# sailist/emotion-recognition-in-conversation

Measured on AMD Instinct MI355X. Metric: utterances/sec training step, COGMEN IEMOCAP-6 atv, higher is better.
Workload: dtype bf16

## Files before the change

### emotion-recognition-in-conversation_amd/capi.py

```python
import ctypes as C
import os
import re
import subprocess

import torch

_HERE = os.path.dirname(os.path.abspath(__file__))
LIB_PATH = os.environ.get("ERC_LIB_PATH") or os.path.join(_HERE, "lib", "libercgraft.so")
CSRC = os.path.join(_HERE, "csrc")
HEADER = os.path.join(os.path.dirname(_HERE), "include", "ercgraft.h")


class ErcGraftError(RuntimeError):
    pass


_CTYPES = {"int": C.c_int, "int32_t": C.c_int, "int64_t": C.c_int64, "uint64_t": C.c_uint64, "float": C.c_float}


def _ctype(decl, proto, ret=False):
    t = " ".join(decl.replace("*", " * ").split())
    if ret and t == "const char *":
        return C.c_char_p
    if "*" in t:
# ... 741 lines not shown


def enc_transpose_bf16(X, ldx, R, Cn, YT, ldyt, plain=None, ldp=0):
    _call("erc_enc_transpose_bf16", X, 1 if X.dtype == torch.float32 else 0, ldx, R, Cn, YT, ldyt, plain, ldp)


def enc_colsum_ws_floats(Cn):
    return int(lib().erc_enc_colsum_ws_floats(Cn))


def enc_colsum(X, ldx, R, Cn, out, ws):
    _call("erc_enc_colsum", X, 1 if X.dtype == torch.bfloat16 else 0, ldx, R, Cn, out, ws)


def enc_inverse_rows(node_row, N, inv, n_rows):
    _call("erc_enc_inverse_rows", node_row, N, inv, n_rows)


def wgrad_bf16(table, n_desc, item_base, n_items, slabs, counters, terms=1):
    if terms > 1:
        _call("erc_wgrad_split", terms, table, n_desc, item_base, n_items, slabs, counters)
        return
    _call("erc_wgrad_bf16", table, n_desc, item_base, n_items, slabs, counters)


def wgrad_bf16_adam(table, n_desc, item_base, n_items, slabs, counters, n_tiles, p, g, m, v, n, lr, b1, b2, eps, wd, decoupled,
                    grad_scale, state, shadow_table, health, terms=1, p2p_desc=None):
    args = (table, n_desc, item_base, n_items, slabs, counters, int(n_tiles), p, g, m, v, n, lr, b1, b2, eps, wd, int(decoupled),
            grad_scale, state) + _shadow(shadow_table)
    if p2p_desc is not None:
        _call("erc_wgrad_adam_p2p", terms, *args, C.addressof(p2p_desc))
    elif terms > 1:
        _call("erc_wgrad_split_adam", terms, *args, health)
    else:
        _call("erc_wgrad_bf16_adam", *args, health)


def wgrad_bf16_wide(table, n_desc, wg_base, n_wgs, slabs, counters):
    _call("erc_wgrad_bf16_wide", table, n_desc, wg_base, n_wgs, slabs, counters)


def wgrad_bf16_set_spin_limit(limit):
    _call("erc_wgrad_bf16_set_spin_limit", int(limit))


def wgrad_bf16_set_stamps(t, item=0):
    _call("erc_wgrad_bf16_set_stamps", t, int(item))


def wgrad_bf16_slab_floats():
    return int(lib().erc_wgrad_bf16_slab_floats())


def wgrad_bf16_max_k_per_split():
    return int(lib().erc_wgrad_bf16_max_k_per_split())


def wgrad_slab_floats():
    return int(lib().erc_wgrad_slab_floats())


def wgrad_max_k_per_split():
    return int(lib().erc_wgrad_max_k_per_split())


def dgcn_tail_limits():
    return int(lib().erc_dgcn_tail_max_rows()), int(lib().erc_dgcn_tail_max_window())


def dgcn_tail_set_stamps(stamps):
    _call("erc_dgcn_tail_set_stamps", stamps)


def dgcn_tail_stats_floats(n_rows):
    return int(lib().erc_dgcn_tail_stats_floats(n_rows))


def dgcn_tail(slabs, n_slabs, slab_stride, rgcn_bias, g, window, W_rel, b_rel, W_root, W1, b1, W2, b2, labels, weight, n_classes,
              n_rows, drop_p, rng, Xc, ldx, Hc, AGG, Zc, logits, dlogits, dZc, dXc, lddx, dAGG, dHc, stats, n_dev=None, label_rows=None):
    args = (slabs, n_slabs, int(slab_stride), rgcn_bias, g["in_ptr"], g["in_src"], window, W_rel, b_rel, W_root, W1, b1, W2, b2,
            labels, weight, n_classes, n_rows, float(drop_p), rng, Xc, ldx, Hc, AGG, Zc, logits, dlogits, dZc, dXc, lddx, dAGG, dHc,
            stats)
    if n_dev is None and label_rows is None:
        _call("erc_dgcn_tail", *args)
    else:
        _call("erc_dgcn_tail_cap", *args, n_dev, label_rows)


def head_ce_stats_floats(n_rows):
    return int(lib().erc_head_ce_stats_floats(n_rows))


def head_ce(Z, ldz, F, Cn, n_rows, W, bias, labels, weight, mask_scale, logits, ldl, dlogits, lddl, dZ, lddz, stats):
    _call("erc_head_ce", Z, ldz, F, Cn, n_rows, W, bias, labels, weight, mask_scale, logits, ldl, dlogits, lddl, dZ, lddz,
          stats)


def cim_meta(lengths, B, T, n_cap, node_off, node_row):
    _call("erc_cim_meta", lengths, B, T, n_cap, node_off, node_row)


def gru_scan_fwd(GX, W_hhT, b_hh, lengths, node_off, B, T, rows, Hout, Hdrop, drop_p, rng, rng_stream, gates, ghn, Hprev):
    _call("erc_gru_scan_fwd", GX, W_hhT, b_hh, lengths, node_off, B, T, rows, Hout, Hdrop, drop_p, rng, rng_stream, gates, ghn,
          Hprev)


# ... 51 lines not shown
```

### emotion-recognition-in-conversation_amd/csrc/wgrad_bf16.hip

```cpp
#include "erc_common.h"
#include "optim_dev.h"
#include "split_dev.h"
#include <string.h>

namespace {

typedef float f32x4 __attribute__((ext_vector_type(4)));
typedef short bf16x8 __attribute__((ext_vector_type(8)));
typedef unsigned int u32x4 __attribute__((ext_vector_type(4)));
typedef unsigned int u32x2 __attribute__((ext_vector_type(2)));
#define ERC_GLOBAL __attribute__((address_space(1)))

constexpr int W2_IDX_CAP = 4096;
constexpr int W2_SLAB = 128 * 64 + 192;
constexpr int W2_MAX_DESC = 16;

struct W2Desc {
    const unsigned short* A;
    const unsigned short* B;
    float* C;
    float* bias_a;
    float* bias_b;
    const int32_t* b_gather;
    const int32_t* k_dev;
    int lda, ldb, ldc, M, N, K;
    int ct, cvec, splits, tiles_n, item_base, n_items, tile_base;
    int kind;
};

struct W2Adam {
    int decoupled, spin_limit;
    float lr, b1, b2, eps, wd, grad_scale;
    float *data, *grad, *m, *v;
    int64_t* state;
    unsigned short* shadow;
    const int32_t* skip;
    int32_t* seq;
    int32_t* health;
    ShadowTab tab;
    int x_world, x_rank, x_spin, x_pad;
    float* x_pub[8];
    int32_t* x_flags[8];
    int64_t* x_epoch;
    int64_t x_npad;
};
static_assert(sizeof(W2Desc) == 112, "W2Desc layout");

__device__ __forceinline__ float ld_sc1(const float* p) { return __hip_atomic_load(p, __ATOMIC_RELAXED, __HIP_MEMORY_SCOPE_AGENT); }
__device__ __forceinline__ void st_sc1(float* p, float v) { __hip_atomic_store(p, v, __ATOMIC_RELAXED, __HIP_MEMORY_SCOPE_AGENT); }
__device__ __forceinline__ void st_sc1_x4(float* p, f32x4 v) {
    asm volatile("global_store_dwordx4 %0, %1, off sc0 sc1\n\ts_nop 1" ::"v"(p), "v"(v) : "memory");
}
__device__ __forceinline__ f32x4 ld_sc1_x4(const float* p) {
    f32x4 v;
    asm volatile("global_load_dwordx4 %0, %1, off sc0 sc1" : "=v"(v) : "v"(p) : "memory");
    return v;
}
__device__ __forceinline__ float bf_lo(unsigned d) { return __builtin_bit_cast(float, d << 16); }
__device__ __forceinline__ float bf_hi(unsigned d) { return __builtin_bit_cast(float, d & 0xffff0000u); }
__device__ __forceinline__ unsigned perm_lo(unsigned x, unsigned y) { return __builtin_amdgcn_perm(y, x, 0x05040100u); }
__device__ __forceinline__ unsigned perm_hi(unsigned x, unsigned y) { return __builtin_amdgcn_perm(y, x, 0x07060302u); }

#define W2_STAMP(slot)                                                                          \
    do {                                                                                        \
        if (stamps && threadIdx.x == 0) stamps[slot] = __builtin_amdgcn_s_memrealtime();        \
    } while (0)

template <bool ADAM, bool WIDE, int NT>
__device__ __forceinline__ void w2_body(const W2Desc& d, const int local, float* red, float* bred, int* idx, int* s_flag,
                                        float* slabs, int* counters, uint64_t* stamps_item, uint64_t* stamps_tile, const W2Adam& ad) {
    uint64_t* stamps = stamps_item;
    W2_STAMP(0);
    bool adam_on = false;
    int64_t adam_step = 0;
    AdamCoef ac;
    if (ADAM && d.kind == 1) {
        const bool skip = ad.skip && __hip_atomic_load(ad.skip, __ATOMIC_RELAXED, __HIP_MEMORY_SCOPE_AGENT) != 0;
        adam_step = ad.state[4 + blockIdx.x] + 1;
        adam_on = !skip;
        ac.init(ad.lr, ad.b1, ad.b2, ad.eps, ad.wd, ad.decoupled, ad.grad_scale, adam_step);
    }
    auto bump_step = [&]() __attribute__((always_inline)) {
        if (!ADAM || !adam_on) return;
        if (threadIdx.x == 0) {
            ad.state[4 + blockIdx.x] = adam_step;
            if (blockIdx.x == 0) ad.state[0] = adam_step, ad.state[1] += 1;
        }
        if (blockIdx.x == 0)
            for (int t = gridDim.x + threadIdx.x; t < 512; t += 256) ad.state[4 + t] = adam_step;
    };
    const ShadowTab& stab = *reinterpret_cast<const ShadowTab*>(red);
    auto copy_tab = [&]() __attribute__((always_inline)) {
        ShadowTab* const wt = reinterpret_cast<ShadowTab*>(red);
        wt->n = ad.tab.n, wt->flags = ad.tab.flags;
#pragma unroll
        for (int t = 0; t < SHADOW_MAX; ++t) {
            const ShadowDesc& a = ad.tab.d[t];
            ShadowDesc& b = wt->d[t];
            b.src_off = a.src_off, b.n_el = a.n_el, b.dst_off = a.dst_off, b.n0 = a.n0, b.n1 = a.n1, b.sn0 = a.sn0, b.sn1 = a.sn1;
            b.sn2 = a.sn2, b.sk0 = a.sk0, b.sk1 = a.sk1, b.sk2 = a.sk2, b.ld = a.ld, b.mode = a.mode;
            b.plane_stride = a.plane_stride, b.terms = a.terms;
        }
    };
    auto adam_quad = [&](const int64_t off, const f32x4 gq, const f32x4 pq, const f32x4 mq, const f32x4 vq) __attribute__((always_inline)) -> float4 {
        float4 pv = make_float4(pq.x, pq.y, pq.z, pq.w), mv = make_float4(mq.x, mq.y, mq.z, mq.w), vv = make_float4(vq.x, vq.y, vq.z, vq.w);
        ac.upd(pv.x, gq.x, mv.x, vv.x), ac.upd(pv.y, gq.y, mv.y, vv.y), ac.upd(pv.z, gq.z, mv.z, vv.z), ac.upd(pv.w, gq.w, mv.w, vv.w);
        *(ERC_GLOBAL f32x4*)(ad.data + off) = (f32x4){pv.x, pv.y, pv.z, pv.w};
        *(ERC_GLOBAL f32x4*)(ad.m + off) = (f32x4){mv.x, mv.y, mv.z, mv.w}, *(ERC_GLOBAL f32x4*)(ad.v + off) = (f32x4){vv.x, vv.y, vv.z, vv.w};
        return pv;
    };
    auto shadow_quads = [&](const int64_t (&offs)[8], const float4 (&pn)[8], const int count, const bool (&isq)[8], const unsigned tmask) __attribute__((always_inline)) {
        if (!ad.shadow) return;
        const bool quads = (stab.flags & 1) != 0;
        const int nt = stab.n;
#pragma unroll
        for (int o = 0; o < 8; ++o) {
            if (o >= count || !isq[o]) continue;
            const int64_t i0 = offs[o];
            const float4 pv = pn[o];
#pragma unroll 1
            for (int t = 0; t < nt; ++t) {
                if (!((tmask >> t) & 1)) continue;
                const ShadowDesc& sd = stab.d[t];
                if (quads) {
                    shadow_store4_desc(ad.shadow, sd, (stab.flags & (2 << t)) != 0, i0, pv);
                } else {
                    shadow_store_desc(ad.shadow, sd, i0, pv.x), shadow_store_desc(ad.shadow, sd, i0 + 1, pv.y);
                    shadow_store_desc(ad.shadow, sd, i0 + 2, pv.z), shadow_store_desc(ad.shadow, sd, i0 + 3, pv.w);
                }
            }
        }
    };
    auto adam_one = [&](const int64_t off, const float gval) __attribute__((always_inline)) {
        float pv = ad.data[off], mv = ad.m[off], vv = ad.v[off];
        ac.upd(pv, gval, mv, vv);
        ad.data[off] = pv, ad.m[off] = mv, ad.v[off] = vv;
        if (ad.shadow) {
            const int nt = stab.n;
#pragma unroll 1
            for (int t = 0; t < nt; ++t) shadow_store_desc(ad.shadow, stab.d[t], off, pv);
        }
    };
    __shared__ int s_x_skip;
    auto x_poff = [&]() __attribute__((always_inline)) -> int64_t { return (int64_t)((ad.x_epoch[blockIdx.x] + 1) & 1) * ad.x_npad; };
    auto x_rendezvous = [&](const bool local_skip) __attribute__((always_inline)) -> bool {
        const int b = blockIdx.x, nblk = gridDim.x;
// ... 3 lines not shown
        if ((int)threadIdx.x < ad.x_world) {
            int32_t *f = nullptr, *mine = nullptr;
#pragma unroll
            for (int r = 0; r < 8; ++r) {
                if (r == (int)threadIdx.x) f = ad.x_flags[r];
                if (r == ad.x_rank) mine = ad.x_flags[r];
            }
            __hip_atomic_store(f + ad.x_rank * nblk + b, ep * 2 + (local_skip ? 1 : 0), __ATOMIC_RELAXED, __HIP_MEMORY_SCOPE_SYSTEM);
            const int32_t* w_ = mine + (int)threadIdx.x * nblk + b;
            int val = __hip_atomic_load(w_, __ATOMIC_RELAXED, __HIP_MEMORY_SCOPE_SYSTEM), spins = 0;
            while ((val >> 1) - ep < 0) {
                if (++spins > ad.x_spin) {
                    __hip_atomic_store(ad.health, ERC_HEALTH_RAISED, __ATOMIC_RELAXED, __HIP_MEMORY_SCOPE_AGENT);
                    val = 2 * ep + 1;
                    break;
                }
                __builtin_amdgcn_s_sleep(2);
                val = __hip_atomic_load(w_, __ATOMIC_RELAXED, __HIP_MEMORY_SCOPE_SYSTEM);
            }
            const unsigned long long any = __ballot((val & 1) != 0);
            if (threadIdx.x == 0) s_x_skip = any != 0ull;
        }
        __syncthreads();
        if (threadIdx.x == 0) ad.x_epoch[b] = ep;
        return s_x_skip == 0;
    };
    auto x_sum4 = [&](const int64_t poff_off) __attribute__((always_inline)) -> f32x4 {
        f32x4 part[8];
#pragma unroll
        for (int r = 0; r < 8; ++r) part[r] = r < ad.x_world ? ld_sc1_x4(ad.x_pub[r] + poff_off) : (f32x4){0.f, 0.f, 0.f, 0.f};
        asm volatile("s_waitcnt vmcnt(0)"
                     : "+v"(part[0]), "+v"(part[1]), "+v"(part[2]), "+v"(part[3]), "+v"(part[4]), "+v"(part[5]), "+v"(part[6]), "+v"(part[7])
                     :
                     : "memory");
        f32x4 acc = {0.f, 0.f, 0.f, 0.f};
#pragma unroll
        for (int r = 0; r < 8; ++r)
            if (r < ad.x_world) acc += part[r];
        return acc;
    };
    auto x_sum1 = [&](const int64_t poff_off) __attribute__((always_inline)) -> float {
        float acc = 0.f;
        for (int r = 0; r < ad.x_world; ++r) {
            const float* pb = nullptr;
#pragma unroll
            for (int q = 0; q < 8; ++q)
                if (q == r) pb = ad.x_pub[q];
            acc += __hip_atomic_load(pb + poff_off, __ATOMIC_RELAXED, __HIP_MEMORY_SCOPE_SYSTEM);
        }
        return acc;
    };
    if (ADAM && d.kind == 1) {
        if (threadIdx.x == 64) copy_tab();
        __syncthreads();
        const int64_t base = d.C - ad.grad;
        int64_t xoff = 0;
        if (ad.x_world > 1) {
            xoff = x_poff() + base;
            float* mypub = nullptr;
#pragma unroll
            for (int r = 0; r < 8; ++r)
                if (r == ad.x_rank) mypub = ad.x_pub[r];
            for (int e = (int)threadIdx.x; e < d.M; e += 256) __hip_atomic_store(mypub + xoff + e, d.C[e], __ATOMIC_RELAXED, __HIP_MEMORY_SCOPE_SYSTEM);
            adam_on = x_rendezvous(!adam_on) && adam_on;
        }
        bump_step();
        if (adam_on) {
            for (int e = 4 * (int)threadIdx.x; e < d.M; e += 1024) {
                if (e + 3 < d.M && ((base + e) & 3) == 0) {
                    int64_t offs[8] = {base + e};
                    float4 pn[8];
                    const bool isq[8] = {true};
                    f32x4 gq = *(const ERC_GLOBAL f32x4*)(d.C + e);
                    if (ad.x_world > 1) {
                        gq = x_sum4(xoff + e);
                        *(ERC_GLOBAL f32x4*)(d.C + e) = gq;
                    }
                    pn[0] = adam_quad(base + e, gq, *(const ERC_GLOBAL f32x4*)(ad.data + base + e),
                                      *(const ERC_GLOBAL f32x4*)(ad.m + base + e), *(const ERC_GLOBAL f32x4*)(ad.v + base + e));
                    shadow_quads(offs, pn, 1, isq, ~0u);
                } else {
                    for (int t = e; t < min(e + 4, d.M); ++t) {
                        float gv = d.C[t];
                        if (ad.x_world > 1) d.C[t] = gv = x_sum1(xoff + t);
                        adam_one(base + t, gv);
                    }
                }
            }
        }
        return;
    }
    const int tid = threadIdx.x, lane = tid & 63, w = tid >> 6, r = lane & 15, g = lane >> 4;
    const int split = local % d.splits;
    const int tn = WIDE ? 4 * (local / d.splits) + w : local / d.splits;
    const int n0 = tn * 64;
    const int nks = (d.K + 3) >> 2;
    const int per = (nks + d.splits - 1) / d.splits;
    const int ks_begin = split * per, ks_end = min(nks, ks_begin + per);
    const int k_begin = ks_begin * 4;
    const int nk = max(1, min(d.K, ks_end * 4) - k_begin);
    const int K_true = d.k_dev ? min(*(const ERC_GLOBAL int32_t*)d.k_dev, d.K) : d.K;
    const ERC_GLOBAL int32_t* const gather = (const ERC_GLOBAL int32_t*)d.b_gather;
    const bool gath = gather != nullptr;
    const ERC_GLOBAL unsigned short* const Ag = (const ERC_GLOBAL unsigned short*)d.A;
    const ERC_GLOBAL unsigned short* const Bg = (const ERC_GLOBAL unsigned short*)d.B;

    auto mrow = [](const int rp, const int i) __attribute__((always_inline)) -> int {
        return NT == 1 ? 8 * rp + i : (i < 4 ? 4 * rp + i : 64 + 4 * rp + (i - 4));
    };
    const int ma = NT == 1 ? 8 * r : 4 * r, nb = n0 + 4 * r;
    const int a_c = ma < d.M ? ma : 0;
    const int b_c = nb < d.N ? nb : 0;
    const int ns = WIDE ? max(0, ks_end - ks_begin) : (max(0, ks_end - ks_begin) + 3) >> 2;
    auto kstep = [&](const int sidx) __attribute__((always_inline)) { return WIDE ? ks_begin + sidx : ks_begin + w + 4 * sidx; };

    f32x4 acc[8][4];
#pragma unroll
    for (int i = 0; i < 8; ++i)
#pragma unroll
        for (int j = 0; j < 4; ++j) acc[i][j] = (f32x4){0.f, 0.f, 0.f, 0.f};
    f32x4 bacc_a[8], bacc_b[4];
#pragma unroll
    for (int i = 0; i < 8; ++i) bacc_a[i] = (f32x4){0.f, 0.f, 0.f, 0.f};
#pragma unroll
    for (int j = 0; j < 4; ++j) bacc_b[j] = (f32x4){0.f, 0.f, 0.f, 0.f};
    const bf16x8 ones = __builtin_bit_cast(bf16x8, (u32x4){0x3F803F80u, 0x3F803F80u, 0x3F803F80u, 0x3F803F80u});
    const bool want_a = d.bias_a != nullptr && tn == 0, want_b = d.bias_b != nullptr;

    if constexpr (NT == 1) {
        auto load_a = [&](const int s0, u32x4 (&a)[8]) {
    #pragma unroll
            for (int u = 0; u < 8; ++u) {
                const int k = 4 * kstep(s0 + u) + g;
                const int kl = max(0, min(k - k_begin, nk - 1));
                a[u] = *(const ERC_GLOBAL u32x4*)(Ag + (int64_t)(k_begin + kl) * d.lda + a_c);
            }
        };
        auto load_b = [&](const int s0, u32x2 (&b)[8]) {
    #pragma unroll
            for (int u = 0; u < 8; ++u) {
                const int k = 4 * kstep(s0 + u) + g;
                const int kl = max(0, min(k - k_begin, nk - 1));
// ... 225 lines not shown
                        if (m + i < d.M) dst[i] = v[i];
                }
            }
        };
    #pragma unroll
        for (int P = 0; P < 2; ++P) {
            __syncthreads();
    #pragma unroll
            for (int hh = 0; hh < 2; ++hh)
    #pragma unroll
                for (int il = 0; il < 2; ++il)
    #pragma unroll
                    for (int q = 0; q < 4; ++q) {
                        const int h = 2 * P + hh;
                        const f32x4 v_n = (f32x4){acc[2 * h + il][0][q], acc[2 * h + il][1][q], acc[2 * h + il][2][q], acc[2 * h + il][3][q]};
                        const f32x4 v_t = (f32x4){acc[4 * il][h][q], acc[4 * il + 1][h][q], acc[4 * il + 2][h][q], acc[4 * il + 3][h][q]};
                        const f32x4 v = ct ? v_t : v_n;
                        *reinterpret_cast<f32x4*>(red + w * 4096 + (((hh * 2 + il) * 4 + q) * 64 + lane) * 4) = v * wsel;
                    }
            __syncthreads();
    #pragma unroll
            for (int u = 0; u < 4; ++u) {
                const int f4 = tid + 256 * u;
                f32x4 s = *reinterpret_cast<const f32x4*>(red + f4 * 4);
    #pragma unroll
                for (int ww = 1; ww < 4; ++ww) {
                    const f32x4 t = *reinterpret_cast<const f32x4*>(red + ww * 4096 + f4 * 4);
                    s += t;
                }
                if (direct) {
                    store_c(tid + 256 * (u & 1), 2 * P + (u >> 1), s);
                } else {
                    st_sc1_x4(slab + ((4 * P + u) * 256 + tid) * 4, s);
                }
            }
        }
        if (tid < 192) {
            const float v = ((bred[tid] + bred[192 + tid]) + bred[384 + tid]) + bred[576 + tid];
            if (direct) {
                if (tid < 128) {
                    if (want_a && tid < d.M) ((ERC_GLOBAL float*)d.bias_a)[tid] = v;
                } else if (want_b && n0 + tid - 128 < d.N) {
                    ((ERC_GLOBAL float*)d.bias_b)[n0 + tid - 128] = v;
                }
            } else {
                st_sc1(slab + 8192 + tid, v);
            }
        }
        W2_STAMP(3);
        if (direct) return;
        if (ADAM) {
            const int S = d.splits, lgS = 31 - __builtin_clz(S), owned = 8 >> lgS;
            const int64_t cbase = d.C - ad.grad;
            asm volatile("s_waitcnt vmcnt(0)" ::: "memory");
            __syncthreads();
            W2_STAMP(4);
            int* const counter = counters + d.tile_base + tn;
            int seq = 0;
            if (tid == 0) {
                seq = ad.seq[blockIdx.x] + 1;
                ad.seq[blockIdx.x] = seq;
                __hip_atomic_fetch_add(counter, 1, __ATOMIC_RELAXED, __HIP_MEMORY_SCOPE_AGENT);
            }
            if (tid == 64) copy_tab();
            int64_t off[8];
            int valid[8];
            f32x4 pq[8], mq[8], vq[8];
    #pragma unroll
            for (int o = 0; o < 8; ++o) {
                const int x = split + (o << lgS);
                valid[o] = 0;
                off[o] = cbase;
                if (o < owned) {
                    int vl;
                    const int64_t a = cbase + quad_addr(tid + 256 * (x & 1), x >> 1, vl);
                    valid[o] = (vl == 4 && d.cvec) ? 4 : -vl;
                    if (vl) off[o] = a;
                    const int64_t oc = valid[o] == 4 ? a : cbase;
                    pq[o] = *(const ERC_GLOBAL f32x4*)(ad.data + oc), mq[o] = *(const ERC_GLOBAL f32x4*)(ad.m + oc), vq[o] = *(const ERC_GLOBAL f32x4*)(ad.v + oc);
                }
            }
            float* bdst = nullptr;
            if (split == 0 && tid < 192) {
                if (tid < 128) {
                    if (want_a && tid < d.M) bdst = d.bias_a + tid;
                } else if (want_b && n0 + tid - 128 < d.N) {
                    bdst = d.bias_b + (n0 + tid - 128);
                }
            }
            const int64_t boff = bdst ? bdst - ad.grad : cbase;
            float bp = ad.data[boff], bm = ad.m[boff], bv = ad.v[boff];
            const bool skip = ad.skip && __hip_atomic_load(ad.skip, __ATOMIC_RELAXED, __HIP_MEMORY_SCOPE_AGENT) != 0;
            adam_step = ad.state[4 + blockIdx.x] + 1;
            adam_on = !skip;
            ac.init(ad.lr, ad.b1, ad.b2, ad.eps, ad.wd, ad.decoupled, ad.grad_scale, adam_step);
            if (tid == 0) {
                int ok = 1, spins = 0;
                while (__hip_atomic_load(counter, __ATOMIC_RELAXED, __HIP_MEMORY_SCOPE_AGENT) - S * seq < 0) {
                    if (++spins >= ad.spin_limit) {
                        __hip_atomic_store(ad.health, ERC_HEALTH_RAISED, __ATOMIC_RELAXED, __HIP_MEMORY_SCOPE_AGENT);
                        ok = 0;
                        break;
                    }
                    __builtin_amdgcn_s_sleep(1);
                }
                *s_flag = ok;
            }
            __syncthreads();
            W2_STAMP(5);
            if (ad.x_world <= 1) bump_step();
            if (!*s_flag) return;
            stamps = stamps_tile ? stamps_tile : stamps;
            W2_STAMP(8);
            const float* const tile_slabs = slabs + (int64_t)(d.item_base + tn * S) * W2_SLAB;
            f32x4 part[8];
    #pragma unroll
            for (int L = 0; L < 8; ++L) {
                const int x = split + ((L >> lgS) << lgS), jx = L & (S - 1);
                part[L] = ld_sc1_x4(tile_slabs + (int64_t)jx * W2_SLAB + (x * 256 + tid) * 4);
            }
            float bt[8];
    #pragma unroll
            for (int jj = 0; jj < 8; ++jj) bt[jj] = split == 0 ? ld_sc1(tile_slabs + (int64_t)min(jj, S - 1) * W2_SLAB + 8192 + (tid < 192 ? tid : 0)) : 0.f;
            asm volatile("s_waitcnt vmcnt(0)"
                         : "+v"(part[0]), "+v"(part[1]), "+v"(part[2]), "+v"(part[3]), "+v"(part[4]), "+v"(part[5]), "+v"(part[6]), "+v"(part[7])
                         :
                         : "memory");
            const f32x4 z = (f32x4){0.f, 0.f, 0.f, 0.f};
            f32x4 res[8];
            if (S == 1) {
    #pragma unroll
                for (int o = 0; o < 8; ++o) res[o] = z + part[o];
            } else if (S == 2) {
    #pragma unroll
                for (int o = 0; o < 8; ++o) res[o] = o < 4 ? (z + part[2 * (o & 3)]) + part[2 * (o & 3) + 1] : z;
            } else if (S == 4) {
    #pragma unroll
                for (int o = 0; o < 8; ++o) res[o] = o < 2 ? (((z + part[4 * (o & 1)]) + part[4 * (o & 1) + 1]) + part[4 * (o & 1) + 2]) + part[4 * (o & 1) + 3] : z;
            } else {
                res[0] = (((((((z + part[0]) + part[1]) + part[2]) + part[3]) + part[4]) + part[5]) + part[6]) + part[7];
    #pragma unroll
                for (int o = 1; o < 8; ++o) res[o] = z;
            }
            W2_STAMP(9);
            float bsum = 0.f;
#pragma unroll
            for (int jj = 0; jj < 8; ++jj) bsum += bt[jj] * (jj < S ? 1.f : 0.f);
            if (ad.x_world > 1) {
                const int64_t poff = x_poff();
                float* mypub = nullptr;
#pragma unroll
                for (int r = 0; r < 8; ++r)
                    if (r == ad.x_rank) mypub = ad.x_pub[r];
#pragma unroll
                for (int o = 0; o < 8; ++o)
                    if (o < owned && valid[o] == 4) st_sc1_x4(mypub + poff + off[o], res[o]);
                if (bdst) __hip_atomic_store(mypub + poff + boff, bsum, __ATOMIC_RELAXED, __HIP_MEMORY_SCOPE_SYSTEM);
                adam_on = x_rendezvous(!adam_on) && adam_on;
                bump_step();
                if (adam_on) {
#pragma unroll
                    for (int o = 0; o < 8; ++o)
                        if (o < owned && valid[o] == 4) res[o] = x_sum4(poff + off[o]);
                    if (bdst) bsum = x_sum1(poff + boff);
                }
            }
            const bool upd = adam_on;
            unsigned tmask = 0;
            {
                const int64_t lo = cbase, hi = cbase + (int64_t)(ct ? d.N : d.M) * d.ldc;
                const int nt = stab.n;
                for (int t = 0; t < nt; ++t)
                    if (stab.d[t].src_off < hi && stab.d[t].src_off + stab.d[t].n_el > lo) tmask |= 1u << t;
            }
    #pragma unroll 1
            for (int it = 0; it < owned; ++it) {
                if (valid[0] == 4) {
                    *(ERC_GLOBAL f32x4*)(ad.grad + off[0]) = res[0];
                    if (upd) {
                        const float4 pv = adam_quad(off[0], res[0], pq[0], mq[0], vq[0]);
                        if (it == 0) W2_STAMP(13);
                        if (ad.shadow) {
                            const int nt = stab.n;
    #pragma unroll 1
                            for (int t = 0; t < nt; ++t) {
                                if (!((tmask >> t) & 1)) continue;
                                shadow_store4_desc(ad.shadow, stab.d[t], (stab.flags & (2 << t)) != 0, off[0], pv);
                            }
                        }
                    }
                } else if (valid[0] != 0) {
                    __hip_atomic_store(ad.health, ERC_HEALTH_RAISED, __ATOMIC_RELAXED, __HIP_MEMORY_SCOPE_AGENT);
                }
                if (it < 2) W2_STAMP(11 + it);
    #pragma unroll
                for (int o = 0; o < 7; ++o)
                    res[o] = res[o + 1], pq[o] = pq[o + 1], mq[o] = mq[o + 1], vq[o] = vq[o + 1], off[o] = off[o + 1], valid[o] = valid[o + 1];
            }
            if (bdst) {
                const float v = bsum;
                *(ERC_GLOBAL float*)bdst = v;
                if (upd) {
                    ac.upd(bp, v, bm, bv);
                    ad.data[boff] = bp, ad.m[boff] = bm, ad.v[boff] = bv;
                    if (ad.shadow) {
                        const int nt = stab.n;
    #pragma unroll 1
                        for (int t = 0; t < nt; ++t) shadow_store_desc(ad.shadow, stab.d[t], boff, bp);
                    }
                }
            }
            W2_STAMP(10);
            return;
        }

        asm volatile("s_waitcnt vmcnt(0)" ::: "memory");
        __syncthreads();
        W2_STAMP(4);
        int* const counter = counters + d.tile_base + tn;
        if (tid == 0) {
            const int prev = __hip_atomic_fetch_add(counter, 1, __ATOMIC_RELAXED, __HIP_MEMORY_SCOPE_AGENT);
            const int last = prev == d.splits - 1;
            if (last) __hip_atomic_store(counter, 0, __ATOMIC_RELAXED, __HIP_MEMORY_SCOPE_AGENT);
            *s_flag = last;
        }
        __syncthreads();
        W2_STAMP(5);
        if (!*s_flag) return;
        stamps = stamps_tile;
        W2_STAMP(8);
        const float* const tile_slabs = slabs + (int64_t)(d.item_base + tn * d.splits) * W2_SLAB;
        f32x4 sum[8];
    #pragma unroll
        for (int x = 0; x < 8; ++x) sum[x] = (f32x4){0.f, 0.f, 0.f, 0.f};
        for (int sp0 = 0; sp0 < d.splits; sp0 += 4) {
            f32x4 v[4][8];
    #pragma unroll
            for (int j = 0; j < 4; ++j) {
                const float* p = tile_slabs + (int64_t)min(sp0 + j, d.splits - 1) * W2_SLAB + tid * 4;
    #pragma unroll
                for (int x = 0; x < 8; ++x) v[j][x] = ld_sc1_x4(p + x * 1024);
            }
    #pragma unroll
            for (int jj = 0; jj < 4; jj += 2)
                asm volatile("s_waitcnt vmcnt(0)"
                             : "+v"(v[jj][0]), "+v"(v[jj][1]), "+v"(v[jj][2]), "+v"(v[jj][3]), "+v"(v[jj][4]), "+v"(v[jj][5]), "+v"(v[jj][6]),
                               "+v"(v[jj][7]), "+v"(v[jj + 1][0]), "+v"(v[jj + 1][1]), "+v"(v[jj + 1][2]), "+v"(v[jj + 1][3]),
                               "+v"(v[jj + 1][4]), "+v"(v[jj + 1][5]), "+v"(v[jj + 1][6]), "+v"(v[jj + 1][7])
                             :
                             : "memory");
    #pragma unroll
            for (int j = 0; j < 4; ++j) {
                const float mk = sp0 + j < d.splits ? 1.f : 0.f;
    #pragma unroll
                for (int x = 0; x < 8; ++x) sum[x] += v[j][x] * mk;
            }
        }
        W2_STAMP(9);
    #pragma unroll
        for (int x = 0; x < 8; ++x) store_c(tid + 256 * (x & 1), x >> 1, sum[x]);
        if (tid < 192) {
            float v = 0.f;
            for (int sp0 = 0; sp0 < d.splits; sp0 += 8) {
                float t[8];
    #pragma unroll
                for (int j = 0; j < 8; ++j) t[j] = ld_sc1(tile_slabs + (int64_t)min(sp0 + j, d.splits - 1) * W2_SLAB + 8192 + tid);
    #pragma unroll
                for (int j = 0; j < 8; ++j) v += t[j] * (sp0 + j < d.splits ? 1.f : 0.f);
            }
            if (tid < 128) {
                if (want_a && tid < d.M) ((ERC_GLOBAL float*)d.bias_a)[tid] = v;
            } else if (want_b && n0 + tid - 128 < d.N) {
                ((ERC_GLOBAL float*)d.bias_b)[n0 + tid - 128] = v;
            }
        }
        W2_STAMP(10);
    };
    if (!WIDE) {
        finish(tn, 1.f);
    } else {
        const int tg = 4 * (local / d.splits);
        for (int t = 0; t < 4 && tg + t < d.tiles_n; ++t) {
            if (t) __syncthreads();
            finish(tg + t, w == t ? 1.f : 0.f);
        }
    }
}

struct W2Bases {
    int v[W2_MAX_DESC];
};

template <bool ADAM, bool WIDE, int NT>
__global__ __launch_bounds__(256) void wgrad_bf16_kernel(const W2Desc* __restrict__ table, const int n_desc, const W2Bases bases,
                                                         float* slabs, int* counters, uint64_t* stamps, int stamp_item, const W2Adam ad) {
    __shared__ __attribute__((aligned(16))) float red[4 * 4096];
    __shared__ float bred[4 * 192];
    __shared__ int idx[W2_IDX_CAP];
    __shared__ int s_flag;
    const int L = blockIdx.x;
    int di = 0;
#pragma unroll
    for (int t = 1; t < W2_MAX_DESC; ++t)
        if (t < n_desc && L >= bases.v[t]) di = t;
    const W2Desc d = table[di];
    const int local = L - bases.v[di];
    if (local >= d.n_items) return;
    const bool st_item = stamps && L == stamp_item, st_tile = stamps && di == 0 && local / d.splits == stamp_item / d.splits;
    w2_body<ADAM, WIDE, NT>(d, local, red, bred, idx, &s_flag, slabs, counters, st_item ? stamps : nullptr, st_tile ? stamps : nullptr, ad);
}

}

static uint64_t* g_w2_stamps = nullptr;
static int g_w2_stamp_item = 0;
extern "C" int erc_wgrad_bf16_set_stamps(uint64_t* stamps, int item) {
    g_w2_stamps = stamps, g_w2_stamp_item = item;
    return ERC_OK;
}
extern "C" int64_t erc_wgrad_bf16_slab_floats(void) { return W2_SLAB; }
extern "C" int erc_wgrad_bf16_max_k_per_split(void) { return W2_IDX_CAP; }

static int g_w2_spin_limit = 2000000;
extern "C" int erc_wgrad_bf16_set_spin_limit(int limit) {
    g_w2_spin_limit = limit > 0 ? limit : 2000000;
    return ERC_OK;
}

static int w2_launch(int mode, const void* table, int n_desc, const int32_t* item_base, int n_items, float* slabs, int32_t* counters,
                     const W2Adam& ad, void* stream, int terms = 1) {
    ERC_REQUIRE(table && item_base && n_desc > 0 && n_desc <= W2_MAX_DESC && n_items > 0 && slabs && counters,
                "wgrad_bf16: bad arguments (at most %d records per launch)", W2_MAX_DESC);
    W2Bases bases{};
    for (int t = 0; t < n_desc; ++t) {
        ERC_REQUIRE(item_base[t] >= 0 && item_base[t] < n_items && (t == 0 ? item_base[0] == 0 : item_base[t] > item_base[t - 1]),
                    "wgrad_bf16: item_base[%d] = %d", t, item_base[t]);
        bases.v[t] = item_base[t];
    }
    ERC_REQUIRE(terms >= 1 && terms <= 3 && (terms == 1 || mode != 2), "wgrad_split: terms = %d (1 .. 3; the wide form is bf16 only)", terms);
#define W2_GO(ADAM_, NT_)                                                                                                              \
    hipLaunchKernelGGL((wgrad_bf16_kernel<ADAM_, false, NT_>), dim3(n_items), dim3(256), 0, (hipStream_t)stream, (const W2Desc*)table, \
                       n_desc, bases, slabs, counters, g_w2_stamps, g_w2_stamp_item, ad)
    if (terms == 2) {
        if (mode == 1) W2_GO(true, 2);
        else W2_GO(false, 2);
    } else if (terms == 3) {
        if (mode == 1) W2_GO(true, 3);
        else W2_GO(false, 3);
    } else if (mode == 1)
        hipLaunchKernelGGL((wgrad_bf16_kernel<true, false, 1>), dim3(n_items), dim3(256), 0, (hipStream_t)stream, (const W2Desc*)table, n_desc,
                           bases, slabs, counters, g_w2_stamps, g_w2_stamp_item, ad);
    else if (mode == 2)
        hipLaunchKernelGGL((wgrad_bf16_kernel<false, true, 1>), dim3(n_items), dim3(256), 0, (hipStream_t)stream, (const W2Desc*)table, n_desc,
                           bases, slabs, counters, g_w2_stamps, g_w2_stamp_item, ad);
    else
        hipLaunchKernelGGL((wgrad_bf16_kernel<false, false, 1>), dim3(n_items), dim3(256), 0, (hipStream_t)stream, (const W2Desc*)table, n_desc,
                           bases, slabs, counters, g_w2_stamps, g_w2_stamp_item, ad);
#undef W2_GO
    ERC_LAUNCH_CHECK("wgrad_bf16");
    return ERC_OK;
}

extern "C" int erc_wgrad_bf16(const void* table, int n_desc, const int32_t* item_base, int n_items, float* slabs,
                              int32_t* counters, void* stream) {
    W2Adam ad{};
// ... 86 lines not shown
```

### emotion-recognition-in-conversation_amd/engine.py

```python
import math
import os

import torch

from . import capi

ALIGN = 64


class WorkspaceCache:

    def __init__(self, maxsize=None):
        import collections
        self.maxsize = int(os.environ.get("ERC_WS_CACHE", 4)) if maxsize is None else maxsize
        self._d = collections.OrderedDict()
        self.last = None

    def get(self, key, make):
        ws = self._d.get(key)
        if ws is None:
            ws = make()
            self._d[key] = ws
            while len(self._d) > self.maxsize:
                victim = next((k for k in self._d if k != key), None)
# ... 227 lines not shown
        fuse = fuse and not wide
        if cache.get("w16_key") != key:
            cap = capi.wgrad_bf16_max_k_per_split()
            tiles = sum(-(-d[7] // 64) for d in self.deferred16)
            if wide:
                tiles = sum(-(-(-(-d[7] // 64)) // 4) for d in self.deferred16)
            K = max(d[8] for d in self.deferred16)
            rows = int(os.environ.get("ERC_W2_ROWS", 1024))
            n_cu_all = min(256, torch.cuda.get_device_properties(self.device).multi_processor_count) if torch.cuda.is_available() else 256
            s_max = max(1, min(32, n_cu_all // tiles, -(-K // 64)))
            groups = lambda sp: -(-(-(-(-(-K // 4) // sp) // 4)) // 8)
            cand = [sp for sp in (1, 2, 4, 8) if sp <= s_max] if fuse else range(1, s_max + 1)
            splits = min(cand, key=lambda sp: (groups(sp), sp))
            splits = max(splits, min(32, -(-K // rows)), -(-K // cap))
            if wide:
                splits = max(-(-K // cap), max(1, min(32, 256 // tiles)))
            raw, items, n_tiles, bases, sps, whole_quads, wgs = [], 0, 0, [], set(), True, 0
            for a, lda, b, ldb, c, ldc, M, N, Kr, ct, ba, bb, g, kd in self.deferred16:
                nks = -(-Kr // 4)
                per = -(-nks // splits)
                sp = -(-nks // per)
                if per * 4 > cap:
                    raise capi.ErcGraftError("bf16 wgrad: K=%d needs more than %d splits" % (Kr, splits))
                tn = -(-N // 64)
                cvec = int(c.data_ptr() % 16 == 0 and ldc % 4 == 0)
                n_wg = -(-tn // 4) * sp if wide else tn * sp
                raw.append(struct.pack("<QQQQQQQ14i", a.data_ptr(), b.data_ptr(), c.data_ptr(),
                                       ba.data_ptr() if ba is not None else 0, bb.data_ptr() if bb is not None else 0,
                                       g.data_ptr() if g is not None else 0, kd.data_ptr() if kd is not None else 0,
                                       lda, ldb, ldc, M, N, Kr, int(ct), cvec, sp, tn, items, n_wg, n_tiles, 0))
                bases.append(wgs if wide else items)
                wgs += n_wg
                sps.add(sp)
                whole_quads = whole_quads and bool(cvec) and (M if ct else N) % 4 == 0
                items += tn * sp
                n_tiles += tn
            n_cu = min(256, torch.cuda.get_device_properties(self.device).multi_processor_count) if torch.cuda.is_available() else 256
            fused = fuse and items + len(self.ranges16) <= n_cu and sps <= {1, 2, 4, 8} and whole_quads
            if fused:
                for r in self.ranges16:
                    raw.append(struct.pack("<QQQQQQQ14i", 0, 0, r.data_ptr(), 0, 0, 0, 0, 0, 0, 0, r.numel(), 0, 0, 0, 0, 1, 1,
                                           items, 1, n_tiles, 1))
                    bases.append(items)
                    items += 1
            cache["w16_fused"] = fused
            cache["w16_tiles"] = n_tiles
            cache["w16_records"] = len(raw)
            cache["w16_table"] = torch.frombuffer(bytearray(b"".join(raw)), dtype=torch.uint8).to(self.device)
            cache["w16_slabs"] = torch.empty(items * capi.wgrad_bf16_slab_floats(), dtype=torch.float32, device=self.device)
            cache["w16_counters"] = torch.zeros(n_tiles + 512, dtype=torch.int32, device=self.device)
            cache["w16_items"] = wgs if wide else items
            cache["w16_bases"] = (ctypes.c_int32 * len(bases))(*bases)
            cache["w16_key"] = key
        if fuse and cache["w16_fused"]:
            f = opt.flat
            capi.wgrad_bf16_adam(cache["w16_table"], cache["w16_records"], cache["w16_bases"], cache["w16_items"], cache["w16_slabs"],
                                 cache["w16_counters"], cache["w16_tiles"], f.data, f.grad, f.exp_avg, f.exp_avg_sq, f.numel, opt.lr, opt.betas[0],
                                 opt.betas[1], opt.eps, opt.weight_decay, opt.decoupled, 1.0 / p2p.world if p2p is not None else 1.0,
                                 opt.state, opt.shadow_table, opt.skip_flag, terms=terms, p2p_desc=p2p.desc if p2p is not None else None)
            self.adam_fused = True
            return
        if wide:
            capi.wgrad_bf16_wide(cache["w16_table"], cache["w16_records"], cache["w16_bases"], cache["w16_items"], cache["w16_slabs"],
                                 cache["w16_counters"])
        else:
            capi.wgrad_bf16(cache["w16_table"], cache["w16_records"], cache["w16_bases"], cache["w16_items"], cache["w16_slabs"],
                            cache["w16_counters"], terms=terms)

    def split_for(self, M, N, K, bk=None, min_chunks=None):
        if N <= 1025 and bk is None:
            return 1
        bk = bk or self.BK
        min_chunks = self.MIN_CHUNKS if min_chunks is None else min_chunks
        tiles = -(-N // 32) * -(-M // 64)
        nchunk = -(-K // bk)
        want = max(1, -(-self.TARGET_WG // tiles))
        return max(1, min(want, self.MAX_SPLIT, nchunk // min_chunks if nchunk >= min_chunks else 1))

    def take(self, n):
        start = (self.cursor + ALIGN - 1) // ALIGN * ALIGN
        if start + n > self.ws.numel():
            raise capi.ErcGraftError("slab workspace too small (%d + %d > %d)" % (start, n, self.ws.numel()))
        self.cursor = start + n
        return start

    def add_job(self, src, stride, S, numel, dst_off):
        self.jobs.append((src, stride, S, numel, dst_off))
        self.max_numel = max(self.max_numel, numel)

    def job_table(self):
        return torch.tensor(self.jobs, dtype=torch.int64, device=self.device)

    def reduce_into(self, cache, grad):
        self.flush_wgrads(cache)
        self.flush_wgrads_bf16(cache)
        if not self.jobs:
            return
        if cache.get("jobs") is None or cache["jobs"].shape[0] != len(self.jobs):
            cache["jobs"] = self.job_table()
        capi.slab_reduce_batched(self.ws, grad, cache["jobs"], len(self.jobs), self.max_numel)


def linear_fwd(pl, x, ldx, gather, W, bias, out, ldo, M, N, K, act=0, drop_p=0.0, rng=None, x_bf16=False, ldw=None):
    ldw = K if ldw is None else ldw
    if x_bf16:
        assert act in (0, 1)
        capi.gemm_bf16a_stream(x, ldx, gather, W, ldw, out, ldo, M, N, K, bias=bias, act=act)
        return
    S = pl.split_for(M, N, K)
    if S == 1:
        capi.gemm_f32(x, ldx, 0, gather, W, ldw, 0, None, out, ldo, M, N, K, bias=bias, act=act,
                      act_scale=(1.0 / (1.0 - drop_p) if act == 3 else 1.0), drop_p=drop_p, rng_state=rng)
    else:
        assert act in (0, 1)
# ... 243 lines not shown
```

### include/ercgraft.h

```cpp
#ifndef ERCGRAFT_H
#define ERCGRAFT_H

#include <stdint.h>

#ifdef __cplusplus
extern "C" {
#endif

#define ERC_ABI_VERSION 3

#define ERC_OK 0
#define ERC_E_ARG (-1)
#define ERC_E_LAUNCH (-2)

int erc_abi_version(void);
const char* erc_last_error(void);

int erc_window_graph_build(const int64_t* lengths, const int64_t* speakers, int64_t spk_sb, int64_t spk_st,
                           int B, int T, int wp, int wf, int n_speakers, int n_cap, int e_cap,
                           int32_t* node_off, int32_t* node_row, int32_t* node_spk,
                           int32_t* in_ptr, int32_t* in_src, int32_t* in_typ,
                           int32_t* out_ptr, int32_t* out_dst, int32_t* out_typ, int32_t* out_eid,
                           int64_t* edge_index, int64_t* edge_type, int32_t* counts, void* stream);
int erc_window_graph_build_desc(const int64_t* lengths, const int64_t* speakers, int64_t spk_sb, int64_t spk_st,
                                int B, int T, int wp, int wf, int n_speakers, int n_cap, int e_cap,
                                int32_t* node_off, int32_t* node_row, int32_t* node_spk,
                                int32_t* in_ptr, int32_t* in_src, int32_t* in_typ,
                                int32_t* out_ptr, int32_t* out_dst, int32_t* out_typ, int32_t* out_eid,
                                int64_t* edge_index, int64_t* edge_type, int32_t* counts, const int32_t* desc, void* stream);

int erc_gemm_f32(const float* A, int lda, int a_kmajor, const int32_t* a_gather,
                 const float* B, int ldb, int b_kmajor, const int32_t* b_gather,
                 float* C, int ldc, int M, int N, int K,
                 int split_k, int64_t c_slab, int ones_col, float* bias_out, int64_t bias_slab,
                 const float* bias, int act, const float* aux, int ldaux, float act_scale,
                 float drop_p, const uint64_t* rng_state, int accumulate, void* stream);

int erc_gemm_f32_stream(const float* A, int lda, int a_kmajor, const int32_t* a_gather,
                        const float* B, int ldb, int b_kmajor, const int32_t* b_gather,
                        float* C, int ldc, int M, int N, int K,
                        int split_k, int64_t c_slab, int ones_col, float* bias_out, int64_t bias_slab,
                        const float* bias, int act, const float* aux, int ldaux, float act_scale,
                        float drop_p, const uint64_t* rng_state, int accumulate, void* stream);
int erc_wgrad_table(const void* table, int n_desc, const int32_t* item_base, int n_items, float* slabs,
                    int32_t* counters, void* stream);
int64_t erc_wgrad_slab_floats(void);
int erc_wgrad_table_x3(const void* table, int n_desc, const int32_t* item_base, int n_items, float* slabs,
                       int32_t* counters, void* stream);
int erc_wgrad_bf16(const void* table, int n_desc, const int32_t* item_base, int n_items, float* slabs, int32_t* counters,
                   void* stream);
int erc_wgrad_bf16_set_spin_limit(int limit);
int erc_wgrad_bf16_wide(const void* table, int n_desc, const int32_t* wg_base, int n_wgs, float* slabs, int32_t* counters,
                        void* stream);
int64_t erc_wgrad_bf16_slab_floats(void);
int erc_wgrad_bf16_set_stamps(uint64_t* stamps, int item);
int erc_wgrad_bf16_max_k_per_split(void);
int erc_wgrad_max_k_per_split(void);

int erc_gemm_bf16a_stream(const void* X, int ldx, const int32_t* gather, const void* W, int ldw, int w_is_bf16,
                          float* C, int ldc, int M, int N, int K, const float* bias, int act, void* stream);

int erc_gemm_bf16x(const void* A, int lda, int a_kmajor, const int32_t* a_gather,
                   const void* B, int ldb, int b_kmajor, const int32_t* b_gather, int x_is_a,
                   float* C, int ldc, int M, int N, int K,
                   int split_k, int64_t c_slab, int ones_col, float* bias_out, int64_t bias_slab,
                   void* stream);

int erc_gemm_x3(const float* A, int lda, const float* B, int ldb, float* C, int ldc, int M, int N, int K, int split_k,
                int64_t c_slab, void* stream);

int erc_gemm_x3_grouped(const float* A, int lda, const float* B, int ldb, float* C, int pitch, const int32_t* node_off,
                        int n_dlg, int n_mod, int n_nodes, int max_rows, int K, int split_k, int64_t c_slab, void* stream);

int erc_slab_reduce(const float* slabs, int S, int64_t slab_stride, const float* bias, int n_cols, int act,
                    float* out, int ld_out, int64_t numel, void* stream);

int erc_slab_reduce_batched(const float* ws, float* dst, const int64_t* jobs, int n_jobs, int64_t max_numel,
                            void* stream);

int erc_rgcn_mean_fwd(const float* x, int ldx, int F, int R, int N,
                      const int32_t* in_ptr, const int32_t* in_src, const int32_t* in_typ,
                      float* Mout, int ldm, float* inv_cnt, void* stream);
int erc_rgcn_mean_bwd(const float* dM, int ldm, int F, int R, int N,
                      const int32_t* out_ptr, const int32_t* out_dst, const int32_t* out_typ,
                      const float* inv_cnt, float* dx, int lddx, void* stream);

int erc_tconv_attn_fwd(const float* qkvs, int ld, int F, int N, float scale,
                       const int32_t* in_ptr, const int32_t* in_src,
                       float* out, int ldo, float* alpha, void* stream);
int erc_tconv_attn_bwd_target(const float* qkvs, int ld, int F, int N, float scale,
                              const int32_t* in_ptr, const int32_t* in_src, const float* alpha,
                              const float* dout, int lddo, float* dqkvs, float* dscore,
                              const float* bn_x, int bn_ldx, const float* bn_gamma, const float* bn_saved,
                              const float* bn_bwd, float* dout_store, void* stream);
int erc_tconv_attn_bwd_source(const float* qkvs, int ld, int F, int N,
                              const int32_t* out_ptr, const int32_t* out_dst, const int32_t* out_eid,
                              const float* alpha, const float* dscore, const float* dout, int lddo,
                              float* dqkvs, void* stream);

int64_t erc_bn_ws_floats(int F);
int erc_bn_lrelu_fwd(const float* x, int ldx, int N, int F, const float* gamma, const float* beta,
                     float* running_mean, float* running_var, float momentum, float eps, float slope,
                     int training, float* saved, float* y, int ldy, float* ws, void* stream);
int erc_bn_lrelu_bwd(const float* x, int ldx, int N, int F, const float* gamma, const float* beta,
                     const float* saved, float slope, const float* dy, int lddy,
                     float* dx, int lddx, float* dgamma, float* dbeta, float* ws, void* stream);

// ... 382 lines not shown
```

Measured before the change: 21.29 million.

## Replace split-K counter spin with sentinel-armed slab polling in fused bf16 wgrad Adam

The fused wgrad+Adam epilogue no longer waits for every split's counter before loading partial slabs. Slabs are pre-filled with a sentinel word, each consumer polls its own quads and re-reads only the ones that still hold the sentinel, then re-arms them after use. Adam coefficients are computed once per block by one wave and shared through LDS, and the per-block skip, step and seq loads are hoisted to kernel entry. This removes the full vmcnt drain, barrier and counter spin, at the cost of a one-time arm kernel and re-arm stores, and it relies on real gradient values never equalling the sentinel bit pattern.

Measured after the change: 21.39 million, median of 4. No clear change (+0.5%).

```diff
diff --git a/emotion-recognition-in-conversation_amd/capi.py b/emotion-recognition-in-conversation_amd/capi.py
--- a/emotion-recognition-in-conversation_amd/capi.py
+++ b/emotion-recognition-in-conversation_amd/capi.py
@@ -817,6 +817,14 @@
     return int(lib().erc_wgrad_bf16_slab_floats())
 
 
+def wgrad_bf16_arm(slabs):
+    _call("erc_wgrad_bf16_arm", slabs, slabs.numel())
+
+
+def wgrad_bf16_arm_word():
+    return int(lib().erc_wgrad_bf16_arm_word())
+
+
 def wgrad_bf16_max_k_per_split():
     return int(lib().erc_wgrad_bf16_max_k_per_split())
 
diff --git a/emotion-recognition-in-conversation_amd/csrc/wgrad_bf16.hip b/emotion-recognition-in-conversation_amd/csrc/wgrad_bf16.hip
--- a/emotion-recognition-in-conversation_amd/csrc/wgrad_bf16.hip
+++ b/emotion-recognition-in-conversation_amd/csrc/wgrad_bf16.hip
@@ -14,6 +14,7 @@
 constexpr int W2_IDX_CAP = 4096;
 constexpr int W2_SLAB = 128 * 64 + 192;
 constexpr int W2_MAX_DESC = 16;
+constexpr unsigned W2_ARM = 0xFFA5C3E1u;
 
 struct W2Desc {
     const unsigned short* A;
@@ -71,14 +72,21 @@
                                         float* slabs, int* counters, uint64_t* stamps_item, uint64_t* stamps_tile, const W2Adam& ad) {
     uint64_t* stamps = stamps_item;
     W2_STAMP(0);
+    if (ADAM && threadIdx.x == 0) *s_flag = 1;
+    int seq = 0, skip_word = 0;
+    int64_t step_prev = 0;
+    if (ADAM) {
+        seq = __builtin_amdgcn_readfirstlane(ad.seq[blockIdx.x]) + 1;
+        if (ad.skip) skip_word = __builtin_amdgcn_readfirstlane(__hip_atomic_load(ad.skip, __ATOMIC_RELAXED, __HIP_MEMORY_SCOPE_AGENT));
+        const int64_t st = ad.state[4 + blockIdx.x];
+        step_prev = ((int64_t)__builtin_amdgcn_readfirstlane((int)(st >> 32)) << 32) | (unsigned)__builtin_amdgcn_readfirstlane((int)st);
+    }
     bool adam_on = false;
     int64_t adam_step = 0;
     AdamCoef ac;
-    if (ADAM && d.kind == 1) {
-        const bool skip = ad.skip && __hip_atomic_load(ad.skip, __ATOMIC_RELAXED, __HIP_MEMORY_SCOPE_AGENT) != 0;
-        adam_step = ad.state[4 + blockIdx.x] + 1;
-        adam_on = !skip;
-        ac.init(ad.lr, ad.b1, ad.b2, ad.eps, ad.wd, ad.decoupled, ad.grad_scale, adam_step);
+    if (ADAM) {
+        adam_step = step_prev + 1;
+        adam_on = skip_word == 0;
     }
     auto bump_step = [&]() __attribute__((always_inline)) {
         if (!ADAM || !adam_on) return;
@@ -89,9 +97,17 @@
         if (blockIdx.x == 0)
             for (int t = gridDim.x + threadIdx.x; t < 512; t += 256) ad.state[4 + t] = adam_step;
     };
-    const ShadowTab& stab = *reinterpret_cast<const ShadowTab*>(red);
+    const ShadowTab& stab = *reinterpret_cast<const ShadowTab*>(idx);
+    static_assert(sizeof(ShadowTab) <= 1024 && sizeof(AdamCoef) == 32, "LDS layout of the table and the coefficients");
+    AdamCoef* const s_coef = reinterpret_cast<AdamCoef*>(idx + 256);
+    auto share_coef = [&]() __attribute__((always_inline)) {
+        if ((threadIdx.x >> 6) != 2) return;
+        AdamCoef c;
+        c.init(ad.lr, ad.b1, ad.b2, ad.eps, ad.wd, ad.decoupled, ad.grad_scale, adam_step);
+        if (threadIdx.x == 128) *s_coef = c;
+    };
     auto copy_tab = [&]() __attribute__((always_inline)) {
-        ShadowTab* const wt = reinterpret_cast<ShadowTab*>(red);
+        ShadowTab* const wt = reinterpret_cast<ShadowTab*>(idx);
         wt->n = ad.tab.n, wt->flags = ad.tab.flags;
 #pragma unroll
         for (int t = 0; t < SHADOW_MAX; ++t) {
@@ -201,7 +217,9 @@
     };
     if (ADAM && d.kind == 1) {
         if (threadIdx.x == 64) copy_tab();
+        share_coef();
         __syncthreads();
+        ac = *s_coef;
         const int64_t base = d.C - ad.grad;
         int64_t xoff = 0;
         if (ad.x_world > 1) {
@@ -237,6 +255,7 @@
                 }
             }
         }
+        W2_STAMP(10);
         return;
     }
     const int tid = threadIdx.x, lane = tid & 63, w = tid >> 6, r = lane & 15, g = lane >> 4;
@@ -568,16 +587,12 @@
         if (ADAM) {
             const int S = d.splits, lgS = 31 - __builtin_clz(S), owned = 8 >> lgS;
             const int64_t cbase = d.C - ad.grad;
-            asm volatile("s_waitcnt vmcnt(0)" ::: "memory");
-            __syncthreads();
-            W2_STAMP(4);
             int* const counter = counters + d.tile_base + tn;
-            int seq = 0;
             if (tid == 0) {
-                seq = ad.seq[blockIdx.x] + 1;
                 ad.seq[blockIdx.x] = seq;
                 __hip_atomic_fetch_add(counter, 1, __ATOMIC_RELAXED, __HIP_MEMORY_SCOPE_AGENT);
             }
+            W2_STAMP(4);
             if (tid == 64) copy_tab();
             int64_t off[8];
             int valid[8];
@@ -606,42 +621,88 @@
             }
             const int64_t boff = bdst ? bdst - ad.grad : cbase;
             float bp = ad.data[boff], bm = ad.m[boff], bv = ad.v[boff];
-            const bool skip = ad.skip && __hip_atomic_load(ad.skip, __ATOMIC_RELAXED, __HIP_MEMORY_SCOPE_AGENT) != 0;
-            adam_step = ad.state[4 + blockIdx.x] + 1;
-            adam_on = !skip;
-            ac.init(ad.lr, ad.b1, ad.b2, ad.eps, ad.wd, ad.decoupled, ad.grad_scale, adam_step);
-            if (tid == 0) {
-                int ok = 1, spins = 0;
-                while (__hip_atomic_load(counter, __ATOMIC_RELAXED, __HIP_MEMORY_SCOPE_AGENT) - S * seq < 0) {
-                    if (++spins >= ad.spin_limit) {
-                        __hip_atomic_store(ad.health, ERC_HEALTH_RAISED, __ATOMIC_RELAXED, __HIP_MEMORY_SCOPE_AGENT);
-                        ok = 0;
-                        break;
-                    }
-                    __builtin_amdgcn_s_sleep(1);
-                }
-                *s_flag = ok;
-            }
-            __syncthreads();
-            W2_STAMP(5);
-            if (ad.x_world <= 1) bump_step();
-            if (!*s_flag) return;
-            stamps = stamps_tile ? stamps_tile : stamps;
-            W2_STAMP(8);
-            const float* const tile_slabs = slabs + (int64_t)(d.item_base + tn * S) * W2_SLAB;
+            float* const tile_slabs = slabs + (int64_t)(d.item_base + tn * S) * W2_SLAB;
+            auto quad_ptr = [&](const int L) __attribute__((always_inline)) -> float* {
+                const int x = split + ((L >> lgS) << lgS), jx = L & (S - 1);
+                return tile_slabs + (int64_t)jx * W2_SLAB + (x * 256 + tid) * 4;
+            };
+            auto unarmed = [](const f32x4 v) __attribute__((always_inline)) -> bool {
+                const u32x4 u = __builtin_bit_cast(u32x4, v);
+                return u.x != W2_ARM && u.y != W2_ARM && u.z != W2_ARM && u.w != W2_ARM;
+            };
+            const bool bown = split == 0 && tid < 192;
+            auto bias_ptr = [&](const int jj) __attribute__((always_inline)) -> float* { return tile_slabs + (int64_t)jj * W2_SLAB + 8192 + tid; };
             f32x4 part[8];
     #pragma unroll
-            for (int L = 0; L < 8; ++L) {
-                const int x = split + ((L >> lgS) << lgS), jx = L & (S - 1);
-                part[L] = ld_sc1_x4(tile_slabs + (int64_t)jx * W2_SLAB + (x * 256 + tid) * 4);
-            }
+            for (int L = 0; L < 8; ++L) part[L] = ld_sc1_x4(quad_ptr(L));
             float bt[8];
     #pragma unroll
-            for (int jj = 0; jj < 8; ++jj) bt[jj] = split == 0 ? ld_sc1(tile_slabs + (int64_t)min(jj, S - 1) * W2_SLAB + 8192 + (tid < 192 ? tid : 0)) : 0.f;
+            for (int jj = 0; jj < 8; ++jj) bt[jj] = 0.f;
+            if (bown) {
+    #pragma unroll
+                for (int jj = 0; jj < 8; ++jj)
+                    if (jj < S) bt[jj] = ld_sc1(bias_ptr(jj));
+            }
+            int cnt = tid == 0 ? __hip_atomic_load(counter, __ATOMIC_RELAXED, __HIP_MEMORY_SCOPE_AGENT) : 0;
+            share_coef();
+            auto missing = [&](const unsigned of) __attribute__((always_inline)) -> unsigned {
+                unsigned ms = 0;
+    #pragma unroll
+                for (int L = 0; L < 8; ++L)
+                    if (((of >> L) & 1) && !unarmed(part[L])) ms |= 1u << L;
+    #pragma unroll
+                for (int jj = 0; jj < 8; ++jj)
+                    if (((of >> (8 + jj)) & 1) && __builtin_bit_cast(unsigned, bt[jj]) == W2_ARM) ms |= 0x100u << jj;
+                if (((of >> 16) & 1) && cnt - S * seq < 0) ms |= 0x10000u;
+                return ms;
+            };
             asm volatile("s_waitcnt vmcnt(0)"
                          : "+v"(part[0]), "+v"(part[1]), "+v"(part[2]), "+v"(part[3]), "+v"(part[4]), "+v"(part[5]), "+v"(part[6]), "+v"(part[7])
                          :
                          : "memory");
+            const unsigned wanted = 0xffu | (bown ? ((1u << S) - 1u) << 8 : 0u) | (tid == 0 ? 0x10000u : 0u);
+            unsigned miss = missing(wanted);
+            int spins = 0, rereq = 0;
+            while (miss) {
+                if (++spins >= ad.spin_limit) {
+                    __hip_atomic_store(ad.health, ERC_HEALTH_RAISED, __ATOMIC_RELAXED, __HIP_MEMORY_SCOPE_AGENT);
+                    *s_flag = 0;
+                    break;
+                }
+                __builtin_amdgcn_s_sleep(4);
+    #pragma unroll
+                for (int L = 0; L < 8; ++L)
+                    if ((miss >> L) & 1) part[L] = ld_sc1_x4(quad_ptr(L)), ++rereq;
+    #pragma unroll
+                for (int jj = 0; jj < 8; ++jj)
+                    if ((miss >> (8 + jj)) & 1) bt[jj] = ld_sc1(bias_ptr(jj));
+                if (miss & 0x10000u) cnt = __hip_atomic_load(counter, __ATOMIC_RELAXED, __HIP_MEMORY_SCOPE_AGENT);
+                asm volatile("s_waitcnt vmcnt(0)"
+                             : "+v"(part[0]), "+v"(part[1]), "+v"(part[2]), "+v"(part[3]), "+v"(part[4]), "+v"(part[5]), "+v"(part[6]), "+v"(part[7])
+                             :
+                             : "memory");
+                miss = missing(miss);
+            }
+            if (stamps && tid == 0) stamps[14] = (uint64_t)rereq, stamps[15] = (uint64_t)spins;
+            auto rearm = [&](const unsigned have) __attribute__((always_inline)) {
+                const f32x4 armq = __builtin_bit_cast(f32x4, (u32x4){W2_ARM, W2_ARM, W2_ARM, W2_ARM});
+    #pragma unroll
+                for (int L = 0; L < 8; ++L)
+                    if ((have >> L) & 1) st_sc1_x4(quad_ptr(L), armq);
+    #pragma unroll
+                for (int jj = 0; jj < 8; ++jj)
+                    if ((have >> (8 + jj)) & 1) st_sc1(bias_ptr(jj), __builtin_bit_cast(float, W2_ARM));
+            };
+            __syncthreads();
+            W2_STAMP(5);
+            ac = *s_coef;
+            if (ad.x_world <= 1) bump_step();
+            if (!*s_flag) {
+                rearm(wanted & ~miss);
+                return;
+            }
+            stamps = stamps_tile ? stamps_tile : stamps;
+            W2_STAMP(8);
             const f32x4 z = (f32x4){0.f, 0.f, 0.f, 0.f};
             f32x4 res[8];
             if (S == 1) {
@@ -726,6 +787,7 @@
                     }
                 }
             }
+            rearm(wanted);
             W2_STAMP(10);
             return;
         }
@@ -812,7 +874,7 @@
                                                          float* slabs, int* counters, uint64_t* stamps, int stamp_item, const W2Adam ad) {
     __shared__ __attribute__((aligned(16))) float red[4 * 4096];
     __shared__ float bred[4 * 192];
-    __shared__ int idx[W2_IDX_CAP];
+    __shared__ __attribute__((aligned(16))) int idx[W2_IDX_CAP];
     __shared__ int s_flag;
     const int L = blockIdx.x;
     int di = 0;
@@ -822,11 +884,29 @@
     const W2Desc d = table[di];
     const int local = L - bases.v[di];
     if (local >= d.n_items) return;
-    const bool st_item = stamps && L == stamp_item, st_tile = stamps && di == 0 && local / d.splits == stamp_item / d.splits;
-    w2_body<ADAM, WIDE, NT>(d, local, red, bred, idx, &s_flag, slabs, counters, st_item ? stamps : nullptr, st_tile ? stamps : nullptr, ad);
-}
-
-}
+    const bool st_all = stamps && stamp_item < 0;
+    uint64_t* const st_mine = st_all ? stamps + 16 * L : stamps;
+    const bool st_item = stamps && (st_all || L == stamp_item);
+    const bool st_tile = stamps && (st_all ? ADAM : di == 0 && local / d.splits == stamp_item / d.splits);
+    w2_body<ADAM, WIDE, NT>(d, local, red, bred, idx, &s_flag, slabs, counters, st_item ? st_mine : nullptr, st_tile ? st_mine : nullptr, ad);
+}
+
+__global__ __launch_bounds__(256) void w2_arm_kernel(u32x4* __restrict__ p, const int64_t n_quads) {
+    for (int64_t i = (int64_t)blockIdx.x * 256 + threadIdx.x; i < n_quads; i += (int64_t)gridDim.x * 256)
+        p[i] = (u32x4){W2_ARM, W2_ARM, W2_ARM, W2_ARM};
+}
+
+}
+
+extern "C" int erc_wgrad_bf16_arm(float* slabs, int64_t n_floats, void* stream) {
+    ERC_REQUIRE(slabs && n_floats > 0 && n_floats % 4 == 0 && ((uintptr_t)slabs & 15) == 0, "wgrad_bf16_arm: bad arguments");
+    const int64_t nq = n_floats / 4;
+    hipLaunchKernelGGL(w2_arm_kernel, dim3((unsigned)((nq + 255) / 256 < 2048 ? (nq + 255) / 256 : 2048)), dim3(256), 0, (hipStream_t)stream,
+                       (u32x4*)slabs, nq);
+    ERC_LAUNCH_CHECK("wgrad_bf16_arm");
+    return ERC_OK;
+}
+extern "C" int erc_wgrad_bf16_arm_word(void) { return (int)W2_ARM; }
 
 static uint64_t* g_w2_stamps = nullptr;
 static int g_w2_stamp_item = 0;
diff --git a/emotion-recognition-in-conversation_amd/engine.py b/emotion-recognition-in-conversation_amd/engine.py
--- a/emotion-recognition-in-conversation_amd/engine.py
+++ b/emotion-recognition-in-conversation_amd/engine.py
@@ -303,14 +303,19 @@
             cache["w16_items"] = wgs if wide else items
             cache["w16_bases"] = (ctypes.c_int32 * len(bases))(*bases)
             cache["w16_key"] = key
+            cache["w16_armed"] = False
         if fuse and cache["w16_fused"]:
             f = opt.flat
+            if not cache.get("w16_armed"):
+                capi.wgrad_bf16_arm(cache["w16_slabs"])
+                cache["w16_armed"] = True
             capi.wgrad_bf16_adam(cache["w16_table"], cache["w16_records"], cache["w16_bases"], cache["w16_items"], cache["w16_slabs"],
                                  cache["w16_counters"], cache["w16_tiles"], f.data, f.grad, f.exp_avg, f.exp_avg_sq, f.numel, opt.lr, opt.betas[0],
                                  opt.betas[1], opt.eps, opt.weight_decay, opt.decoupled, 1.0 / p2p.world if p2p is not None else 1.0,
                                  opt.state, opt.shadow_table, opt.skip_flag, terms=terms, p2p_desc=p2p.desc if p2p is not None else None)
             self.adam_fused = True
             return
+        cache["w16_armed"] = False
         if wide:
             capi.wgrad_bf16_wide(cache["w16_table"], cache["w16_records"], cache["w16_bases"], cache["w16_items"], cache["w16_slabs"],
                                  cache["w16_counters"])
diff --git a/include/ercgraft.h b/include/ercgraft.h
--- a/include/ercgraft.h
+++ b/include/ercgraft.h
@@ -53,6 +53,8 @@
 int erc_wgrad_bf16_wide(const void* table, int n_desc, const int32_t* wg_base, int n_wgs, float* slabs, int32_t* counters,
                         void* stream);
 int64_t erc_wgrad_bf16_slab_floats(void);
+int erc_wgrad_bf16_arm(float* slabs, int64_t n_floats, void* stream);
+int erc_wgrad_bf16_arm_word(void);
 int erc_wgrad_bf16_set_stamps(uint64_t* stamps, int item);
 int erc_wgrad_bf16_max_k_per_split(void);
 int erc_wgrad_max_k_per_split(void);
```
